# freewilll/doom-rust-renderer

Hardware: AMD Instinct MI355X
Metric: frames/sec (fixed e1m1 camera path) (higher is better)
Workload: dtype f32

## Files before the change

doom-rust-renderer_amd/csrc/context.cpp:

```cpp
#include <hip/hip_runtime_api.h>
#include <sched.h>

#include <algorithm>
#include <atomic>
#include <cstdlib>
#include <cstdio>
#include <cstring>
#include <chrono>
#include <memory>
#include <string>
#include <thread>
#include <vector>

#include "../../include/doomgpu.h"
#include "api_common.hpp"
#include "binner.hpp"
#include "fe_kernels.hpp"
#include "fs_kernels.hpp"
#include "light_fx_kernels.hpp"
#include "mobj_fx_kernels.hpp"
#include "frontend.hpp"
#include "hip_mem.hpp"
#include "kernels.hpp"
#include "map_kernels.hpp"
// ... 58 lines not shown
    DevPtr<uint32_t> d_flags;
    FeParams FP{};
    FsParams FSP{};
    LfxRows LR{};
    MfxRows MR{};
    int32_t front_end = DG_FE_HOST;
    void describe(int32_t fe, int n, uint64_t bytes, uint64_t walls, uint64_t planes) {
        front_end = fe; phase = Phase::Prepared; n_frames = n; list_bytes = bytes; n_walls = walls; n_planes = planes;
        max_spans = 0; n_spans = 0; covered = 0;
    }
    bool column_walk() const { return front_end == DG_FE_DEVICE || front_end == DG_FE_DEVICE_SEGS; }
    bool seg_walk() const { return front_end == DG_FE_DEVICE_SEGS; }
    bool harvested = true;
    bool map_built = false;
    std::vector<dg_view> views;
    std::vector<dg_view_state> states;
    std::vector<dg_sector_light> state_lights;
    std::vector<dg_mobj_state> state_mobjs;
    const Scene *snap_scene = nullptr;
    uint64_t snap_rev = 0;
    std::vector<dg_sector_light> snap_lights;
    std::vector<dg_mobj_state> snap_mobjs;
    void snapshot_scene(const Scene &sc) {
        if (snap_scene == &sc && snap_rev == sc.revision && snap_lights.size() == sc.sectors.size() && snap_mobjs.size() == sc.mobjs.size()) return;
        snap_lights.resize(sc.sectors.size()); snap_mobjs.resize(sc.mobjs.size());
        for (size_t i = 0; i < sc.sectors.size(); i++) snap_lights[i] = dg_sector_light{(int32_t)i, (int32_t)sc.sectors[i].light};
        for (size_t i = 0; i < sc.mobjs.size(); i++) snap_mobjs[i] = dg_mobj_state{(int32_t)i, sc.mobjs[i].sprite_frame, sc.mobjs[i].full_bright ? 1 : 0, 0};
        snap_scene = &sc; snap_rev = sc.revision;
    }
    struct RedoState { std::vector<dg_sector_light> lights; std::vector<dg_mobj_state> mobjs; dg_view_state st{}; };
    const dg_view_state *state_for_redo(const Scene &sc, int i, RedoState &tmp, const SceneFx &fx) const {
        const dg_view_state *own = states.empty() ? nullptr : &states[(size_t)i];
        if (snap_scene != &sc || snap_rev == sc.revision) return own;
        tmp.lights.clear();
        const bool lfx = fx.light.fits(sc), mfx = fx.mobj.fits(sc);
        for (const dg_sector_light &l : snap_lights)
            if (!lfx || fx.light.rec_of[(size_t)l.sector] < 0) tmp.lights.push_back(l);
        tmp.mobjs.clear();
        for (const dg_mobj_state &m : snap_mobjs)
            if (!mfx || fx.mobj.type_of[(size_t)m.mobj] < 0) tmp.mobjs.push_back(m);
        if (own) { tmp.lights.insert(tmp.lights.end(), own->lights, own->lights + own->n_lights); tmp.mobjs.insert(tmp.mobjs.end(), own->mobjs, own->mobjs + own->n_mobjs); }
        tmp.st = dg_view_state{tmp.lights.data(), (uint32_t)tmp.lights.size(), tmp.mobjs.data(), (uint32_t)tmp.mobjs.size()};
        return &tmp.st;
    }
    void keep_states(const dg_view_state *st, int n) {
        states.clear(); state_lights.clear(); state_mobjs.clear();
        if (!st) return;
        for (int i = 0; i < n; i++) { state_lights.insert(state_lights.end(), st[i].lights, st[i].lights + st[i].n_lights); state_mobjs.insert(state_mobjs.end(), st[i].mobjs, st[i].mobjs + st[i].n_mobjs); }
        size_t lo = 0, mo = 0;
        for (int i = 0; i < n; i++) {
            states.push_back(dg_view_state{state_lights.data() + lo, st[i].n_lights, state_mobjs.data() + mo, st[i].n_mobjs});
            lo += st[i].n_lights; mo += st[i].n_mobjs;
        }
    }
};

struct FeFrameOut {
    std::vector<FePart> parts;
    std::vector<FeSprite> sprites;
    std::vector<uint32_t> behind, sky_parts, bin_off, sbin_off;
    std::vector<uint16_t> bin_parts, sbin_sprites;
    uint32_t behind_words = 0, n_sky_slots = 0;
    DevFrame hdr{};
};

}

struct dg_ctx {
    dg_config cfg{};
    FrameConsts fk{};
    DevConsts dk{};
    const Scene *scene = nullptr;
    size_t uploaded_texels = 0;
    DevPtr<uint32_t> d_palette;
    DevPtr<uint8_t> d_texel_idx, d_texel_opq;
    uint8_t *d_flats = nullptr;
    DevPtr<unsigned long long> d_checksums;
    DevPtr<uint4> d_row_tab;
    DevScene dscene{};
    std::vector<Slot> slots;
    hipStream_t kstream = nullptr;
    hipStream_t rstream = nullptr;
    bool raster_overlap = false;
    std::unique_ptr<Pool> pool;
    std::vector<std::unique_ptr<FrameArena>> arenas;
    std::vector<BinnedFrame> binned;
    size_t span_cap_per_batch = 0, wall_cap_per_batch = 0, plane_cap_per_batch = 0;
    int n_threads = 1;
    bool fe_enabled = false;
    bool fe_scene_ok = false;
    bool fs_enabled = false, fs_scene_ok = false;
    bool fs_rows_dirty = true;
    bool preparing = false;
    bool fs_forced = false;
    double ema_host = -1.0, ema_gpu_dev = -1.0, ema_gpu_fs = -1.0;
    int host_samples = 0;
    int since_probe = 0;
    int since_fs_probe = 0;
    int gpu_samples[2] = {0, 0};
    DevPtr<uint8_t> d_fs_scene;
    SceneFx fx;
    DevPtr<uint8_t> d_wall_fx;
    FsFx fs_fx{};
    DevPtr<uint8_t> d_light_fx;
    LfxRows lfx_proto{};
    DevPtr<uint8_t> d_mobj_fx;
    MfxRows mfx_proto{};
    DevPtr<uint8_t> d_fs_scratch;
    size_t fs_zero_bytes = 0;
    FsParams fs_proto{};
    uint64_t fallbacks_fe = 0;
    uint64_t redone_frames = 0;
    DevPtr<DevRSpan> d_redo_rspans;
    size_t redo_span_cap = 0;
    std::vector<FeFrameOut> fe_out;
    uint32_t fe_col_slots = FE_DEFAULT_COL_SLOTS;
    size_t fe_part_cap = 0, fe_sprite_cap = 0, fe_behind_cap = 0, fe_bin_cap = 0, fe_sbin_cap = 0, fe_slab_cap = 0;
    DevPtr<uint32_t> d_fe_cnt;
    DevPtr<FeU4> d_fe_cspans;
    DevPtr<FeColRec> d_fe_recs;
    DevPtr<uint8_t> d_map_layer;
    bool map_layer_ok = false;
    DevPtr<uint8_t> d_walk_tables;
    const WalkNode *d_walk_nodes = nullptr;
    const WalkLeaf *d_walk_leaves = nullptr;
    hipStream_t wstream = nullptr;
    hipStream_t xstream = nullptr;
    hipEvent_t ev_reduce0 = nullptr, ev_reduce1 = nullptr;
    bool reduce_timed = false;
};

namespace {

int cgroup_cpu_quota() {
    long long quota = -1, period = 0;
    if (FILE *f = std::fopen("/sys/fs/cgroup/cpu.max", "r")) {
        char q[32] = {0};
        if (std::fscanf(f, "%31s %lld", q, &period) == 2 && std::strcmp(q, "max") != 0) quota = std::atoll(q);
        std::fclose(f);
    } else {
        if (FILE *g = std::fopen("/sys/fs/cgroup/cpu/cpu.cfs_quota_us", "r")) { if (std::fscanf(g, "%lld", &quota) != 1) quota = -1; std::fclose(g); }
        if (FILE *g = std::fopen("/sys/fs/cgroup/cpu/cpu.cfs_period_us", "r")) { if (std::fscanf(g, "%lld", &period) != 1) period = 0; std::fclose(g); }
    }
    if (quota <= 0 || period <= 0) return 0;
    return (int)((quota + period - 1) / period);
}

hipError_t slot_sync(Slot &s) {
    if (s.raster_recorded) { const hipError_t e = hipEventSynchronize(s.ev_raster); if (e != hipSuccess) return e; }
    return hipStreamSynchronize(s.stream);
}

void free_ctx(dg_ctx *c) {
    if (!c) return;
    (void)hipSetDevice(c->cfg.device);
    if (c->kstream) (void)hipStreamSynchronize(c->kstream);
    if (c->rstream) (void)hipStreamSynchronize(c->rstream);
    for (Slot &s : c->slots) {
        if (s.stream) (void)hipStreamSynchronize(s.stream);
        if (s.copy_stream) (void)hipStreamSynchronize(s.copy_stream);
        for (hipEvent_t ev : {s.ev_start, s.ev_setup, s.ev_raster, s.ev_rstart, s.ev_h2d})
            if (ev) (void)hipEventDestroy(ev);
        if (s.copy_stream) (void)hipStreamDestroy(s.copy_stream);
        if (s.stream) (void)hipStreamDestroy(s.stream);
    }
    if (c->kstream) (void)hipStreamDestroy(c->kstream);
    if (c->rstream) (void)hipStreamDestroy(c->rstream);
    if (c->wstream) { (void)hipStreamSynchronize(c->wstream); (void)hipStreamDestroy(c->wstream); }
    if (c->xstream) { (void)hipStreamSynchronize(c->xstream); (void)hipStreamDestroy(c->xstream); }
    for (hipEvent_t ev : {c->ev_reduce0, c->ev_reduce1})
        if (ev) (void)hipEventDestroy(ev);
    delete c;
}

int check_batch(const dg_ctx *c, int n) {
    if (!c->scene) return set_err(DG_ERR_INVALID, "no scene uploaded (dg_upload_scene)");
    if (n <= 0 || n > c->cfg.max_batch) return set_err(DG_ERR_CAPACITY, "batch size outside [1, max_batch]");
    if (c->scene->texel_idx.size() != c->uploaded_texels) return set_err(DG_ERR_INVALID, "the scene decoded new bitmaps since dg_upload_scene: upload it again");
    return DG_OK;
}

void pack_binned(uint8_t *h, const ListLayout &L, const BinnedFrame &bf, size_t i, size_t W) {
    std::memcpy(h + L.frames + i * sizeof(DevFrame), &bf.hdr, sizeof(DevFrame));
    std::memcpy(h + L.col_off + i * (W + 1) * 4, bf.col_off.data(), (W + 1) * 4);
    if (!bf.walls.empty()) std::memcpy(h + L.walls + (size_t)bf.hdr.wall_base * sizeof(DevWallRec), bf.walls.data(), bf.walls.size() * sizeof(DevWallRec));
    if (!bf.planes.empty()) std::memcpy(h + L.planes + (size_t)bf.hdr.plane_base * sizeof(DevPlaneRec), bf.planes.data(), bf.planes.size() * sizeof(DevPlaneRec));
    if (!bf.spans.empty()) std::memcpy(h + L.spans + (size_t)bf.hdr.span_base * sizeof(DevSpan), bf.spans.data(), bf.spans.size() * sizeof(DevSpan));
}

void point_at_lists(RasterParams &P, const uint8_t *d, const ListLayout &L) {
    P.frames = reinterpret_cast<const DevFrame *>(d + L.frames);
    P.col_off = reinterpret_cast<const uint32_t *>(d + L.col_off);
    P.walls = reinterpret_cast<const DevWallRec *>(d + L.walls);
    P.planes = reinterpret_cast<const DevPlaneRec *>(d + L.planes);
    P.spans = reinterpret_cast<const DevSpan *>(d + L.spans);
}

void fill_raster_params(dg_ctx *c, Slot &s, int n) {
    RasterParams &P = s.P;
    P.scene = c->dscene;
    P.k = c->dk;
    P.rspans = s.d_rspans.get();
    P.fb = s.d_fb.get();
    P.row_tab = c->d_row_tab.get();
    P.n_frames = n;
}

template <class T> void point_at(T *&p, uint8_t *d, size_t off) { p = reinterpret_cast<T *>(d + off); }
template <class Params, class Layout> void point_at_records(Params &P, uint8_t *d, const Layout &L) {
    point_at(P.fframes, d, L.fframes); point_at(P.parts, d, L.parts); point_at(P.sprites, d, L.sprites);
    point_at(P.behind, d, L.behind); point_at(P.sky_parts, d, L.sky);
    point_at(P.bin_off, d, L.bin_off); point_at(P.sbin_off, d, L.sbin_off); point_at(P.bin_parts, d, L.bins); point_at(P.sbin_sprites, d, L.sbins);
}

uint32_t fe_span_stride(const dg_ctx *c) { return (uint32_t)(c->span_cap_per_batch / (size_t)c->cfg.max_batch); }

void fill_walk_params(dg_ctx *c, Slot &s, int n) {
    FeParams &F = s.FP;
    F.scene = c->dscene;
    F.k = c->dk;
    F.cspans = c->d_fe_cspans.get(); F.recs = c->d_fe_recs.get(); F.cnt = c->d_fe_cnt.get();
    F.events = s.d_events;
    F.flags = s.d_flags.get();
    F.host_flags = s.h_status.get(); F.totals = s.h_status.get() + c->cfg.max_batch;
    F.col_off = s.d_fe_coloff.get(); F.rspans = s.d_rspans.get();
    F.n_frames = n; F.span_stride = fe_span_stride(c); F.w64 = (uint32_t)((c->cfg.width + 63) / 64); F.col_slots = c->fe_col_slots;
    fill_raster_params(c, s, n);
    s.P.frames = F.frames;
    s.P.col_off = s.d_fe_coloff.get();
    s.P.walls = nullptr; s.P.planes = nullptr; s.P.spans = nullptr;
}

int build_batch_host(dg_ctx *c, Slot &s, const dg_view *views, const dg_frame_lists *given, int n, const dg_view_state *states = nullptr) {
    const auto t0 = std::chrono::steady_clock::now();
    if (const int bad = check_batch(c, n)) return bad;
    const Scene &sc = *c->scene;
    const int W = c->cfg.width, H = c->cfg.height;
    std::vector<int> rc((size_t)n, 0);
    std::vector<std::string> errs((size_t)n);
    c->pool->parallel_for(n, [&](int i, int wid) {
        BinnedFrame &bf = c->binned[(size_t)i];
        if (given) {
            dg_frame_lists fl = given[i];
            fill_view_trig(fl.view);
            rc[(size_t)i] = bin_frame(sc, c->fk, fl, bf, errs[(size_t)i]);
        } else {
            dg_view v = views[i];
            fill_view_trig(v);
            dg_frame_lists fl;
            rc[(size_t)i] = build_frame_lists(sc, W, H, v, *c->arenas[(size_t)wid], fl, errs[(size_t)i], states ? &states[i] : nullptr, &c->fx);
            if (!rc[(size_t)i]) rc[(size_t)i] = bin_frame(sc, c->fk, fl, bf, errs[(size_t)i]);
        }
    });
    for (int i = 0; i < n; i++)
        if (rc[(size_t)i]) return set_err(rc[(size_t)i], "frame " + std::to_string(i) + ": " + errs[(size_t)i]);

    uint64_t spans = 0, walls = 0, planes = 0, covered = 0;
    uint32_t max_spans = 0;
    for (int i = 0; i < n; i++) {
        BinnedFrame &bf = c->binned[(size_t)i];
        bf.hdr.span_base = (uint32_t)spans; bf.hdr.wall_base = (uint32_t)walls; bf.hdr.plane_base = (uint32_t)planes;
        spans += bf.spans.size(); walls += bf.walls.size(); planes += bf.planes.size(); covered += bf.covered_pixels;
        max_spans = std::max<uint32_t>(max_spans, (uint32_t)bf.spans.size());
    }
    if (spans > c->span_cap_per_batch || walls > c->wall_cap_per_batch || planes > c->plane_cap_per_batch)
        return set_err(DG_ERR_CAPACITY, "frame lists exceed the slot's list slab");
    const ListLayout L = list_layout((size_t)n, (size_t)W, walls, planes, spans);
    if (L.total > s.lists_cap) return set_err(DG_ERR_CAPACITY, "list slab too small");
    c->pool->parallel_for(n, [&](int i, int) { pack_binned(s.h_lists.get(), L, c->binned[(size_t)i], (size_t)i, (size_t)W); });
    fill_raster_params(c, s, n);
    point_at_lists(s.P, s.d_lists.get(), L);
    s.describe(DG_FE_HOST, n, L.total, walls, planes);
    s.max_spans = max_spans; s.n_spans = spans; s.covered = covered;
    s.host_ms = std::chrono::duration<float, std::milli>(std::chrono::steady_clock::now() - t0).count();
    HIP_TRY(hipMemcpyAsync(s.d_lists.get(), s.h_lists.get(), L.total, hipMemcpyHostToDevice, s.stream));
    return DG_OK;
}

int build_batch_fe(dg_ctx *c, Slot &s, const dg_view *views, int n, const dg_view_state *states) {
    const auto t0 = std::chrono::steady_clock::now();
    if (const int bad = check_batch(c, n)) return bad;
    const Scene &sc = *c->scene;
    const int W = c->cfg.width, H = c->cfg.height;
    std::vector<int> rc((size_t)n, 0);
    std::vector<std::string> errs((size_t)n);
    c->pool->parallel_for(n, [&](int i, int wid) {
        FrameArena &A = *c->arenas[(size_t)wid];
        FeFrameOut &o = c->fe_out[(size_t)i];
// ... 535 lines not shown
}

}

extern "C" {

int dg_create(const dg_config *cfg, dg_ctx **out) {
    if (!cfg || !out) return set_err(DG_ERR_INVALID, "null argument");
    if (cfg->width <= 0 || cfg->height <= 0 || cfg->width > 16384 || cfg->height > 16384)
        return set_err(DG_ERR_INVALID, "width/height must be positive, both <= 16384");
    if (cfg->max_batch <= 0 || cfg->max_batch > 65535 || cfg->slots <= 0 || cfg->slots > 16)
        return set_err(DG_ERR_INVALID, "max_batch must be in [1, 65535], slots in [1, 16]");
    if (cfg->front_end < DG_FE_AUTO || cfg->front_end > DG_FE_DEVICE_SEGS) return set_err(DG_ERR_INVALID, "front_end must be DG_FE_AUTO, DG_FE_HOST, DG_FE_DEVICE or DG_FE_DEVICE_SEGS");
    int ndev = 0;
    if (hipGetDeviceCount(&ndev) != hipSuccess || ndev <= 0) return set_err(DG_ERR_NO_DEVICE, "no HIP device (this library has no CPU path)");
    if (cfg->device < 0 || cfg->device >= ndev) return set_err(DG_ERR_NO_DEVICE, "device ordinal out of range");
    hipDeviceProp_t prop;
    HIP_TRY(hipGetDeviceProperties(&prop, cfg->device));
    if (std::strncmp(prop.gcnArchName, "gfx950", 6) != 0)
        return set_err(DG_ERR_NO_DEVICE, std::string("device is ") + prop.gcnArchName + ", this build targets gfx950 only");
    HIP_TRY(hipSetDevice(cfg->device));

    dg_ctx *c = new dg_ctx();
    c->cfg = *cfg;
    c->fk = make_consts(cfg->width, cfg->height);
    c->dk = DevConsts{c->fk.ARC, c->fk.GCFX, c->fk.CFX, c->fk.CFY, cfg->width, cfg->height};
    int nthreads = cfg->host_threads;
    if (nthreads <= 0) {
        cpu_set_t set;
        CPU_ZERO(&set);
        int avail = sched_getaffinity(0, sizeof set, &set) == 0 ? CPU_COUNT(&set) : (int)std::thread::hardware_concurrency();
        const int quota = cgroup_cpu_quota();
        if (quota > 0) avail = std::min(avail, quota);
        nthreads = std::max(1, std::min(avail, 16));
    }
    nthreads = std::min(nthreads, 256);
    c->n_threads = nthreads;
    c->pool.reset(new Pool(nthreads - 1));
    for (int i = 0; i < nthreads; i++) c->arenas.emplace_back(new FrameArena());
    c->binned.resize((size_t)cfg->max_batch);

    const size_t W = (size_t)cfg->width, H = (size_t)cfg->height, F = (size_t)cfg->max_batch;
    c->span_cap_per_batch = F * W * 24;
    c->wall_cap_per_batch = F * 4096;
    c->plane_cap_per_batch = F * 4096;
    const size_t lists_cap = list_layout(F, W, c->wall_cap_per_batch, c->plane_cap_per_batch, c->span_cap_per_batch).total + 1024;
    c->fe_enabled = cfg->front_end != DG_FE_HOST;
    c->fs_enabled = cfg->front_end == DG_FE_DEVICE_SEGS || cfg->front_end == DG_FE_AUTO;
    c->fs_forced = cfg->front_end == DG_FE_DEVICE_SEGS;
    if (c->fe_enabled) {
        if (const char *e = std::getenv("DOOMGPU_FE_COLUMN_SLOTS")) {
            const long v = std::strtol(e, nullptr, 10);
            if (v >= 1 && v <= (long)FE_MAX_COL_SLOTS) c->fe_col_slots = (uint32_t)v;
        }
        c->fe_out.resize(F);
        size_t parts_per_frame = 2048;
        if (const char *e = std::getenv("DOOMGPU_FE_RECORDS_PER_FRAME")) {
            const long v = std::strtol(e, nullptr, 10);
            if (v >= 1 && v <= 65535) parts_per_frame = (size_t)v;
        }
        c->fe_part_cap = F * parts_per_frame;
        c->fe_sprite_cap = F * 256;
        c->fe_behind_cap = F * 256 * 32;
        c->fe_bin_cap = F * 16384;
        c->fe_sbin_cap = F * 2048;
        c->fe_slab_cap = fe_layout(F, W, c->fe_part_cap, c->fe_sprite_cap, c->fe_behind_cap, F * FE_MAX_SKY_SLOTS, c->fe_bin_cap, c->fe_sbin_cap).total + 1024;
    }
    c->slots.resize((size_t)cfg->slots);
    hipError_t e;
#define CTX_TRY(expr) if ((e = (expr)) != hipSuccess) { std::string m = std::string(#expr) + ": " + hipGetErrorString(e); free_ctx(c); return set_err(DG_ERR_HIP, m); }
    CTX_TRY(hip_alloc(c->d_checksums, F * 8));
    if (c->fe_enabled) {
        CTX_TRY(hip_alloc(c->d_fe_cspans, F * c->fe_col_slots * W * sizeof(FeU4)));
        CTX_TRY(hip_alloc(c->d_fe_recs, F * c->fe_col_slots * W * sizeof(FeColRec)));
        CTX_TRY(hip_alloc(c->d_fe_cnt, F * W * 4));
    }
    {
        int lo = 0, hi = 0;
        CTX_TRY(hipDeviceGetStreamPriorityRange(&lo, &hi));
        CTX_TRY(hipStreamCreateWithPriority(&c->kstream, hipStreamNonBlocking, hi));
        c->raster_overlap = (size_t)cfg->width * (size_t)cfg->height <= kOverlapMaxPixels;
        if (const char *e = std::getenv("DOOMGPU_RASTER_OVERLAP")) c->raster_overlap = std::atoi(e) != 0;
        if (c->raster_overlap) CTX_TRY(hipStreamCreateWithPriority(&c->rstream, hipStreamNonBlocking, hi));
    }
    for (Slot &s : c->slots) {
        CTX_TRY(hipStreamCreateWithFlags(&s.stream, hipStreamNonBlocking));
        for (hipEvent_t *ev : {&s.ev_start, &s.ev_setup, &s.ev_raster, &s.ev_rstart}) CTX_TRY(hipEventCreate(ev));
        CTX_TRY(hipEventCreateWithFlags(&s.ev_h2d, hipEventDisableTiming));
        CTX_TRY(hipStreamCreateWithFlags(&s.copy_stream, hipStreamNonBlocking));
        CTX_TRY(hip_alloc(s.h_lists, lists_cap));
        CTX_TRY(hip_alloc(s.d_lists, lists_cap));
        CTX_TRY(hip_alloc(s.d_rspans, c->span_cap_per_batch * sizeof(DevRSpan)));
        CTX_TRY(hip_alloc(s.d_fb, F * 3 * W * H));
        if (c->fe_enabled) {
            CTX_TRY(hip_alloc(s.h_fe, c->fe_slab_cap));
            CTX_TRY(hip_alloc(s.d_fe, c->fe_slab_cap));
            CTX_TRY(hip_alloc(s.d_fe_coloff, F * (W + 1) * 4));
            CTX_TRY(hip_alloc(s.d_order, FS_ORDER_CLASSES * F * fe_col_groups(W) * 4));
            SlabCursor ws;
            ws.take(F * 4 + FS_ORDER_CLASSES * 4);
            const size_t off_events = ws.take(F * FE_MAX_SKY_SLOTS * 3 * ((W + 63) / 64) * 8);
            s.walk_state_bytes = ws.end();
            CTX_TRY(hip_alloc(s.d_flags, s.walk_state_bytes));
            s.d_events = reinterpret_cast<uint64_t *>(reinterpret_cast<uint8_t *>(s.d_flags.get()) + off_events);
            CTX_TRY(hip_alloc(s.h_status, 2 * F * 4));
        }
        s.lists_cap = lists_cap;
    }
#undef CTX_TRY
    *out = c;
    return DG_OK;
}

void dg_destroy(dg_ctx *ctx) { free_ctx(ctx); }
int dg_ctx_host_threads(const dg_ctx *ctx) { return ctx ? ctx->n_threads : DG_ERR_INVALID; }

int dg_upload_scene(dg_ctx *c, const dg_scene *scene) {
    if (!c || !scene) return set_err(DG_ERR_INVALID, "null argument");
    HIP_TRY(hipSetDevice(c->cfg.device));
    for (Slot &s : c->slots) {
        if (c->scene) (void)take_slot(c, s);
        HIP_TRY(slot_sync(s));
        HIP_TRY(hipStreamSynchronize(s.copy_stream));
        s.copy_pending = false;
    }
    const Scene &sc = *scene->sc;
    c->d_palette.reset(); c->d_texel_idx.reset(); c->d_texel_opq.reset();
    c->d_flats = nullptr;
    for (Slot &s : c->slots) s.reset();
    c->d_walk_tables.reset();
    c->map_layer_ok = false;
    uint32_t pal[256];
    for (int i = 0; i < 256; i++) pal[i] = (uint32_t)sc.palette[3 * i] | ((uint32_t)sc.palette[3 * i + 1] << 8) | ((uint32_t)sc.palette[3 * i + 2] << 16);
    const size_t nt = std::max<size_t>(sc.texel_idx.size(), 16), nf = std::max<size_t>(sc.flat_pool.size(), 16);
    float palf[256 * 4];
    for (int i = 0; i < 256; i++) { palf[4 * i] = (float)sc.palette[3 * i]; palf[4 * i + 1] = (float)sc.palette[3 * i + 1]; palf[4 * i + 2] = (float)sc.palette[3 * i + 2]; palf[4 * i + 3] = 0.0f; }
    HIP_TRY(hip_alloc(c->d_palette, sizeof pal + sizeof palf));
    const size_t flats_at = (nt + 255) & ~(size_t)255;
    HIP_TRY(hip_alloc(c->d_texel_idx, flats_at + nf));
    HIP_TRY(hip_alloc(c->d_texel_opq, nt));
    c->d_flats = c->d_texel_idx.get() + flats_at;
    HIP_TRY(hipMemcpy(c->d_palette.get(), pal, sizeof pal, hipMemcpyHostToDevice));
    HIP_TRY(hipMemcpy(c->d_palette.get() + 256, palf, sizeof palf, hipMemcpyHostToDevice));
    if (!sc.texel_idx.empty()) {
        HIP_TRY(hipMemcpy(c->d_texel_idx.get(), sc.texel_idx.data(), sc.texel_idx.size(), hipMemcpyHostToDevice));
        HIP_TRY(hipMemcpy(c->d_texel_opq.get(), sc.texel_opq.data(), sc.texel_opq.size(), hipMemcpyHostToDevice));
    }
    if (!sc.flat_pool.empty()) HIP_TRY(hipMemcpy(c->d_flats, sc.flat_pool.data(), sc.flat_pool.size(), hipMemcpyHostToDevice));
    const BitmapInfo &sky = sc.bitmaps[(size_t)sc.sky_bitmap];
    c->dscene = DevScene{c->d_palette.get(), reinterpret_cast<const float *>(c->d_palette.get() + 256), c->d_texel_idx.get(), c->d_texel_opq.get(), c->d_flats, sky.texel_off, sky.w, sky.h, sky.has_holes};
    if (!c->d_row_tab) HIP_TRY(hip_alloc(c->d_row_tab, (size_t)c->cfg.height * sizeof(uint4)));
    HIP_TRY(launch_row_table(c->dscene, c->dk, c->d_row_tab.get(), nullptr));
    HIP_TRY(hipDeviceSynchronize());
    c->scene = &sc;
    c->fx = sc.fx;
    c->fe_scene_ok = sky.w >= 256 && sky.h >= 128;
    c->uploaded_texels = sc.texel_idx.size();
    c->fs_scene_ok = false;
    if (c->fs_enabled && c->fe_scene_ok && sc.fs_ok && c->cfg.width <= FS_MAX_W) {
        const int rc = upload_fs_scene(c, sc);
        if (rc && c->fs_forced) return rc;
        if (rc) {
            static bool said = false;
            if (!said) { said = true; std::fprintf(stderr, "doomgpu: DG_FE_AUTO keeps the per-seg half on the host: no device memory for the seg walk's per-batch rows (%d views x %zu segs)\n", c->cfg.max_batch, sc.segs.size()); }
            drop_fs_scene(c);
            c->fs_scene_ok = false;
// ... 345 lines not shown
```

doom-rust-renderer_amd/csrc/kernels.hip:

```cpp
#include <hip/hip_runtime.h>
#include <cstdlib>
#include <hip/hip_ext.h>

#include <algorithm>
#include <type_traits>

#include "kernels.hpp"
#include "raster_core.h"

namespace dg {

constexpr int TILE_W = 64;
constexpr int TILE_H = 64;
constexpr int WAVES = 8;
constexpr int THREADS = WAVES * 64;
constexpr int SPAN_CAP = 512;

__global__ __launch_bounds__(256) void dg_setup_spans(RasterParams P) {
    const int f = blockIdx.y;
    const DevFrame fr = P.frames[f];
    const uint32_t i = blockIdx.x * blockDim.x + threadIdx.x;
    if (i >= fr.n_spans) return;
    const DevSpan sp = P.spans[fr.span_base + i];
    DevRSpan o;
// ... 411 lines not shown
                C.winner = off;
            } else {
                if (big & colmask) {
                    const uint32_t n0 = bcast(f_n0, 8 * k), n = bcast(f_n, 8 * k);
                    C.winner = big_column_owner(L.lw0 + n0, 32u * (n0 + 1u), n, lane, y0, R);
                } else {
                    C.winner = owner_loop(hit_op & colmask, v_lo, v_rg, v_off, R, 0u);
                }
                o = owner_texel(T, L.lspans, C.winner, R, C.factor);
            }
            C.tex = P.scene.texel_idx[o];
        };
        auto stage2 = [&](int k, const Col &C) {
            const unsigned long long colmask = 0xffull << (8 * k);
            uint32_t tex = C.tex;
            float factor = C.factor;
            if (walk2 & colmask) {
                if (big & colmask) {
                    const uint32_t n0 = bcast(f_n0, 8 * k), n = bcast(f_n, 8 * k);
                    big_column_overlays(P, T, L.lw0 + n0, lspans_addr, 32u * (n0 + 1u), n, lane, y0, R, C.winner, tex, factor);
                } else {
                    overlay_loop(P, T, lspans_addr, hit_ov & colmask, v_lo, v_rg, v_off, R, C.winner, tex, factor);
                }
            }
            float4 c;
            asm volatile("ds_read_b128 %0, %1\n\ts_waitcnt lgkmcnt(0)" : "=v"(c) : "v"(pal_addr + (tex << 4)));
            tcol[k * WAVES * TILE_TS] = shade_f(c, factor);
        };
        Col A, B;
        if (nk == WAVES) {
            stage1(0, A);
#pragma unroll
            for (int k = 1; k < WAVES - 1; k += 2) {
                stage1(k, B);
                stage2(k - 1, A);
                stage1(k + 1, A);
                stage2(k, B);
            }
            stage1(WAVES - 1, B);
            stage2(WAVES - 2, A);
            stage2(WAVES - 1, B);
        } else {
            for (int k = 0; k < nk; k++) {
                stage1(k, A);
                stage2(k, A);
            }
        }

        c_lo = c_hi;
        if (c_lo < TILE_W) __syncthreads();
    }
    __syncthreads();

    const int gc = (lane & 7) | ((lane >> 5) << 3), rsub = (lane >> 3) & 3;
#pragma unroll
    for (int pass = 0; pass < TILE_H / (4 * WAVES); pass++) {
        const int row = pass * 4 * WAVES + wave * 4 + rsub;
        const int yy = y0 + row, xx = x0 + 4 * gc;
        if (yy < H && xx < W) {
            const uint32_t p0 = L.tile[(4 * gc + 0) * TILE_TS + row], p1 = L.tile[(4 * gc + 1) * TILE_TS + row];
            const uint32_t p2 = L.tile[(4 * gc + 2) * TILE_TS + row], p3 = L.tile[(4 * gc + 3) * TILE_TS + row];
            if constexpr (W4) {
                uint32_t *dst = reinterpret_cast<uint32_t *>(fb + ((size_t)yy * (size_t)W + (size_t)xx) * 3);
                __builtin_nontemporal_store((p0 & 0xffffffu) | (p1 << 24), dst + 0);
                __builtin_nontemporal_store(((p1 >> 8) & 0xffffu) | (p2 << 16), dst + 1);
                __builtin_nontemporal_store(((p2 >> 16) & 0xffu) | (p3 << 8), dst + 2);
            } else {
                uint8_t *dst = fb + ((size_t)yy * (size_t)W + (size_t)xx) * 3;
                const uint32_t px[4] = {p0, p1, p2, p3};
#pragma unroll
                for (int j = 0; j < 4; j++) {
                    if (xx + j >= W) break;
                    __builtin_nontemporal_store((uint8_t)px[j], dst + 3 * j + 0);
                    __builtin_nontemporal_store((uint8_t)(px[j] >> 8), dst + 3 * j + 1);
                    __builtin_nontemporal_store((uint8_t)(px[j] >> 16), dst + 3 * j + 2);
                }
            }
        }
    }
    if (ty + 1 < ty_end) __syncthreads();
  }
}

__device__ __forceinline__ void raster_block(const RasterParams &P, uint32_t &bx, uint32_t &by, uint32_t &f) {
    bx = blockIdx.x; by = blockIdx.y; f = blockIdx.z;
    if (!P.frame_per_xcd) return;
    const uint32_t gx = gridDim.x, gy = gridDim.y, pf = gx * gy;
    const uint32_t orig = bx + gx * (by + gy * f);
    if (orig >= ((uint32_t)P.n_frames & ~7u) * pf) return;
    const uint32_t xcd = orig & 7u, idx = orig >> 3;
    const uint32_t j = __umulhi(idx, P.xcd_rcp_pf), w = idx - j * pf;
    f = j * 8u + xcd;
    by = __umulhi(w, P.xcd_rcp_gx);
    bx = w - by * gx;
}

__global__ __launch_bounds__(THREADS, 8) void dg_raster_tiles(RasterParams P) {
    __shared__ __attribute__((aligned(16))) TileLds L;
    const int n_tile_rows = (P.k.H + TILE_H - 1) / TILE_H;
    uint32_t bx, by, f;
    raster_block(P, bx, by, f);
    const int ty_begin = (int)by * P.tile_rows_per_wg;
    strip_body<true>(P, L, (int)f, (int)bx * TILE_W, ty_begin, min(n_tile_rows, ty_begin + P.tile_rows_per_wg));
}
__global__ __launch_bounds__(THREADS, 8) void dg_raster_tiles_anyw(RasterParams P) {
    __shared__ __attribute__((aligned(16))) TileLds L;
    const int n_tile_rows = (P.k.H + TILE_H - 1) / TILE_H;
    uint32_t bx, by, f;
    raster_block(P, bx, by, f);
    const int ty_begin = (int)by * P.tile_rows_per_wg;
    strip_body<false>(P, L, (int)f, (int)bx * TILE_W, ty_begin, min(n_tile_rows, ty_begin + P.tile_rows_per_wg));
}

__global__ void dg_row_table(DevScene scene, DevConsts k, uint4 *row_tab) {
    const int y = (int)(blockIdx.x * blockDim.x + threadIdx.x);
    if (y >= k.H) return;
    const float vy = k.CFY - (float)y;
    const int32_t srow = sky_row(scene, k, y);
    row_tab[y] = make_uint4(f32_bits(prepare_rcp(vy)), f32_bits(vy), (srow < 0 ? 0u : (uint32_t)srow) | (vy != 0.0f ? 0x100u : 0u), f32_bits(srow < 0 ? 0.0f : 1.0f));
}

__global__ __launch_bounds__(256) void dg_checksum(const uint8_t *fb, size_t frame_bytes, unsigned long long *out) {
    const uint8_t *b = fb + (size_t)blockIdx.y * frame_bytes;
    const uint32_t *d = reinterpret_cast<const uint32_t *>(b);
    const bool dwords = (frame_bytes & 3) == 0;
    const size_t n = (frame_bytes + 3) / 4;
    unsigned long long acc = 0;
    for (size_t i = (size_t)blockIdx.x * blockDim.x + threadIdx.x; i < n; i += (size_t)gridDim.x * blockDim.x) {
        uint32_t v;
        if (dwords) v = d[i];
        else {
            v = 0;
            for (size_t k = 0; k < 4 && 4 * i + k < frame_bytes; k++) v |= (uint32_t)b[4 * i + k] << (8 * k);
        }
        unsigned long long m = ((unsigned long long)v ^ (i * 0x9E3779B97F4A7C15ull)) * 0xBF58476D1CE4E5B9ull;
        acc += m ^ (m >> 32);
    }
    for (int o = 32; o > 0; o >>= 1) acc += __shfl_down(acc, o);
    if ((threadIdx.x & 63) == 0) atomicAdd(&out[blockIdx.y], acc);
}

hipError_t launch_checksums(const uint8_t *fb, size_t frame_bytes, int count, unsigned long long *out, hipStream_t stream) {
    if (count <= 0) return hipSuccess;
    const unsigned blocks = (unsigned)std::min<size_t>(256, ((frame_bytes + 3) / 4 + 255) / 256);
    hipLaunchKernelGGL(dg_checksum, dim3(blocks, (unsigned)count), dim3(256), 0, stream, fb, frame_bytes, out);
    return hipGetLastError();
}

hipError_t launch_row_table(const DevScene &scene, const DevConsts &k, uint4 *row_tab, hipStream_t stream) {
    hipLaunchKernelGGL(dg_row_table, dim3((unsigned)((k.H + 255) / 256)), dim3(256), 0, stream, scene, k, row_tab);
    return hipGetLastError();
}

static hipError_t record_pair(hipStream_t stream, hipEvent_t start, hipEvent_t stop) {
    hipError_t e = hipSuccess;
    if (start) e = hipEventRecord(start, stream);
    if (e == hipSuccess && stop) e = hipEventRecord(stop, stream);
    return e;
}

hipError_t launch_setup(const RasterParams &P, uint32_t max_spans_per_frame, hipStream_t stream, hipEvent_t start, hipEvent_t stop) {
    if (P.n_frames <= 0 || max_spans_per_frame == 0) return record_pair(stream, start, stop);
    dim3 grid((max_spans_per_frame + 255) / 256, (unsigned)P.n_frames);
    hipExtLaunchKernelGGL(dg_setup_spans, grid, dim3(256), 0, stream, start, stop, 0, P);
    return hipGetLastError();
}

int raster_tile_rows_per_wg(int W, int H, int n_frames) {
    const int n_tile_rows = (H + TILE_H - 1) / TILE_H;
    if (n_tile_rows < 8) return std::min(2, n_tile_rows);
    const long long strips = (long long)((W + TILE_W - 1) / TILE_W) * (long long)std::max(1, n_frames);
    long long segments = (30000 + strips - 1) / strips;
    segments = std::max(1ll, std::min(segments, (long long)((n_tile_rows + 2) / 3)));
    return (int)((n_tile_rows + segments - 1) / segments);
}

hipError_t launch_raster(const RasterParams &P_in, hipStream_t stream, hipEvent_t start, hipEvent_t stop) {
    if (P_in.n_frames <= 0) return record_pair(stream, start, stop);
    RasterParams P = P_in;
    const int n_tile_rows = (P.k.H + TILE_H - 1) / TILE_H;
    if (P.tile_rows_per_wg <= 0) P.tile_rows_per_wg = raster_tile_rows_per_wg(P.k.W, P.k.H, P.n_frames);
    dim3 grid((unsigned)((P.k.W + TILE_W - 1) / TILE_W), (unsigned)((n_tile_rows + P.tile_rows_per_wg - 1) / P.tile_rows_per_wg), (unsigned)P.n_frames);
    P.frame_per_xcd = (size_t)P.k.W * (size_t)P.k.H <= 1100000 ? 1 : 0;
    if (const char *e = std::getenv("DOOMGPU_FRAME_PER_XCD")) P.frame_per_xcd = std::atoi(e) != 0 ? 1 : 0;
    {
        const uint64_t gx = grid.x, pf = (uint64_t)grid.x * grid.y, total = pf * grid.z;
        if (gx < 2 || total * pf >= (1ull << 32)) P.frame_per_xcd = 0;
        else { P.xcd_rcp_pf = (uint32_t)((1ull << 32) / pf + 1); P.xcd_rcp_gx = (uint32_t)((1ull << 32) / gx + 1); }
    }
    if (P.k.W % 4 == 0) hipExtLaunchKernelGGL(dg_raster_tiles, grid, dim3(THREADS), 0, stream, start, stop, 0, P);
    else hipExtLaunchKernelGGL(dg_raster_tiles_anyw, grid, dim3(THREADS), 0, stream, start, stop, 0, P);
    return hipGetLastError();
}

}
```

doom-rust-renderer_amd/csrc/kernels.hpp:

```cpp
#pragma once
#include <hip/hip_runtime_api.h>
#include <hip/hip_vector_types.h>

#include "lists_dev.h"

namespace dg {

struct RasterParams {
    DevScene scene;
    DevConsts k;
    const DevFrame *frames;
    const uint32_t *col_off;
    const DevSpan *spans;
    DevRSpan *rspans;
    const DevWallRec *walls;
    const DevPlaneRec *planes;
    uint8_t *fb;
    const uint4 *row_tab;
    int32_t n_frames;
    int32_t frame_per_xcd;
    uint32_t xcd_rcp_pf, xcd_rcp_gx;
    int32_t tile_rows_per_wg;
};

hipError_t launch_setup(const RasterParams &P, uint32_t max_spans_per_frame, hipStream_t stream, hipEvent_t start = nullptr, hipEvent_t stop = nullptr);
hipError_t launch_raster(const RasterParams &P, hipStream_t stream, hipEvent_t start = nullptr, hipEvent_t stop = nullptr);
hipError_t launch_checksums(const uint8_t *fb, size_t frame_bytes, int count, unsigned long long *out, hipStream_t stream);
hipError_t launch_row_table(const DevScene &scene, const DevConsts &k, uint4 *row_tab, hipStream_t stream);

}
```

Baseline: 559,800.

## Split raster grid into full-height long strips plus short tail segments

Replaces the uniform raster work-group mapping with a planner that can give most frames full-height column strips (one work-group per strip) and cut the remaining tail frames into short row segments, dealt across XCDs. The aim is to cut per-work-group overhead on the bulk of frames while keeping the GPU busy at the tail of the batch. The default rule turns the split on whenever the frame count leaves enough long strips. It adds index-decoding arithmetic per block and a debug export, and long strips risk load imbalance.

```diff
diff --git a/doom-rust-renderer_amd/csrc/context.cpp b/doom-rust-renderer_amd/csrc/context.cpp
--- a/doom-rust-renderer_amd/csrc/context.cpp
+++ b/doom-rust-renderer_amd/csrc/context.cpp
@@ -164,6 +164,7 @@
     hipStream_t kstream = nullptr;
     hipStream_t rstream = nullptr;
     bool raster_overlap = false;
+    RasterAsk raster_ask;
     std::unique_ptr<Pool> pool;
     std::vector<std::unique_ptr<FrameArena>> arenas;
     std::vector<BinnedFrame> binned;
@@ -286,6 +287,7 @@
     P.fb = s.d_fb.get();
     P.row_tab = c->d_row_tab.get();
     P.n_frames = n;
+    P.ask = c->raster_ask;
 }
 
 template <class T> void point_at(T *&p, uint8_t *d, size_t off) { p = reinterpret_cast<T *>(d + off); }
@@ -987,6 +989,15 @@
         c->raster_overlap = (size_t)cfg->width * (size_t)cfg->height <= kOverlapMaxPixels;
         if (const char *e = std::getenv("DOOMGPU_RASTER_OVERLAP")) c->raster_overlap = std::atoi(e) != 0;
         if (c->raster_overlap) CTX_TRY(hipStreamCreateWithPriority(&c->rstream, hipStreamNonBlocking, hi));
+        if (const char *e = std::getenv("DOOMGPU_FRAME_PER_XCD")) c->raster_ask.frame_per_xcd = std::atoi(e) != 0 ? 1 : 0;
+        if (const char *e = std::getenv("DOOMGPU_RASTER_SHAPE")) {
+            int n_long = 0, rows = 0;
+            if (!std::strcmp(e, "uniform")) c->raster_ask.shape = 1;
+            else if (!std::strcmp(e, "split")) c->raster_ask.shape = 2;
+            else if (std::sscanf(e, "split:%d:%d", &n_long, &rows) == 2 && n_long >= 0 && rows >= 1) {
+                c->raster_ask.shape = 2; c->raster_ask.n_long = n_long; c->raster_ask.short_rows = rows;
+            }
+        }
     }
     for (Slot &s : c->slots) {
         CTX_TRY(hipStreamCreateWithFlags(&s.stream, hipStreamNonBlocking));
diff --git a/doom-rust-renderer_amd/csrc/kernels.hip b/doom-rust-renderer_amd/csrc/kernels.hip
--- a/doom-rust-renderer_amd/csrc/kernels.hip
+++ b/doom-rust-renderer_amd/csrc/kernels.hip
@@ -517,34 +517,23 @@
   }
 }
 
-__device__ __forceinline__ void raster_block(const RasterParams &P, uint32_t &bx, uint32_t &by, uint32_t &f) {
-    bx = blockIdx.x; by = blockIdx.y; f = blockIdx.z;
-    if (!P.frame_per_xcd) return;
-    const uint32_t gx = gridDim.x, gy = gridDim.y, pf = gx * gy;
-    const uint32_t orig = bx + gx * (by + gy * f);
-    if (orig >= ((uint32_t)P.n_frames & ~7u) * pf) return;
-    const uint32_t xcd = orig & 7u, idx = orig >> 3;
-    const uint32_t j = __umulhi(idx, P.xcd_rcp_pf), w = idx - j * pf;
-    f = j * 8u + xcd;
-    by = __umulhi(w, P.xcd_rcp_gx);
-    bx = w - by * gx;
+__device__ __forceinline__ RasterBlock raster_block(const RasterMap &M) {
+    if (M.split) return raster_map_split(M, blockIdx.x);
+    const uint32_t orig = blockIdx.x + gridDim.x * (blockIdx.y + gridDim.y * blockIdx.z);
+    if (orig < M.b1) return raster_map_dealt(M, orig);
+    const int32_t ty = (int32_t)blockIdx.y * M.rows;
+    return RasterBlock{blockIdx.z, blockIdx.x, ty, min(M.n_tile_rows, ty + M.rows)};
 }
 
 __global__ __launch_bounds__(THREADS, 8) void dg_raster_tiles(RasterParams P) {
     __shared__ __attribute__((aligned(16))) TileLds L;
-    const int n_tile_rows = (P.k.H + TILE_H - 1) / TILE_H;
-    uint32_t bx, by, f;
-    raster_block(P, bx, by, f);
-    const int ty_begin = (int)by * P.tile_rows_per_wg;
-    strip_body<true>(P, L, (int)f, (int)bx * TILE_W, ty_begin, min(n_tile_rows, ty_begin + P.tile_rows_per_wg));
+    const RasterBlock b = raster_block(P.map);
+    strip_body<true>(P, L, (int)b.f, (int)b.bx * TILE_W, b.ty_begin, b.ty_end);
 }
 __global__ __launch_bounds__(THREADS, 8) void dg_raster_tiles_anyw(RasterParams P) {
     __shared__ __attribute__((aligned(16))) TileLds L;
-    const int n_tile_rows = (P.k.H + TILE_H - 1) / TILE_H;
-    uint32_t bx, by, f;
-    raster_block(P, bx, by, f);
-    const int ty_begin = (int)by * P.tile_rows_per_wg;
-    strip_body<false>(P, L, (int)f, (int)bx * TILE_W, ty_begin, min(n_tile_rows, ty_begin + P.tile_rows_per_wg));
+    const RasterBlock b = raster_block(P.map);
+    strip_body<false>(P, L, (int)b.f, (int)b.bx * TILE_W, b.ty_begin, b.ty_end);
 }
 
 __global__ void dg_row_table(DevScene scene, DevConsts k, uint4 *row_tab) {
@@ -601,31 +590,35 @@
     return hipGetLastError();
 }
 
-int raster_tile_rows_per_wg(int W, int H, int n_frames) {
-    const int n_tile_rows = (H + TILE_H - 1) / TILE_H;
-    if (n_tile_rows < 8) return std::min(2, n_tile_rows);
-    const long long strips = (long long)((W + TILE_W - 1) / TILE_W) * (long long)std::max(1, n_frames);
-    long long segments = (30000 + strips - 1) / strips;
-    segments = std::max(1ll, std::min(segments, (long long)((n_tile_rows + 2) / 3)));
-    return (int)((n_tile_rows + segments - 1) / segments);
-}
+int raster_tile_rows_per_wg(int W, int H, int n_frames) { return raster_uniform_rows(W, H, n_frames); }
 
 hipError_t launch_raster(const RasterParams &P_in, hipStream_t stream, hipEvent_t start, hipEvent_t stop) {
     if (P_in.n_frames <= 0) return record_pair(stream, start, stop);
     RasterParams P = P_in;
-    const int n_tile_rows = (P.k.H + TILE_H - 1) / TILE_H;
-    if (P.tile_rows_per_wg <= 0) P.tile_rows_per_wg = raster_tile_rows_per_wg(P.k.W, P.k.H, P.n_frames);
-    dim3 grid((unsigned)((P.k.W + TILE_W - 1) / TILE_W), (unsigned)((n_tile_rows + P.tile_rows_per_wg - 1) / P.tile_rows_per_wg), (unsigned)P.n_frames);
-    P.frame_per_xcd = (size_t)P.k.W * (size_t)P.k.H <= 1100000 ? 1 : 0;
-    if (const char *e = std::getenv("DOOMGPU_FRAME_PER_XCD")) P.frame_per_xcd = std::atoi(e) != 0 ? 1 : 0;
-    {
-        const uint64_t gx = grid.x, pf = (uint64_t)grid.x * grid.y, total = pf * grid.z;
-        if (gx < 2 || total * pf >= (1ull << 32)) P.frame_per_xcd = 0;
-        else { P.xcd_rcp_pf = (uint32_t)((1ull << 32) / pf + 1); P.xcd_rcp_gx = (uint32_t)((1ull << 32) / gx + 1); }
-    }
+    uint32_t g[3];
+    P.map = raster_plan(P.k.W, P.k.H, P.n_frames, P.tile_rows_per_wg, P.ask, g);
+    const dim3 grid(g[0], g[1], g[2]);
     if (P.k.W % 4 == 0) hipExtLaunchKernelGGL(dg_raster_tiles, grid, dim3(THREADS), 0, stream, start, stop, 0, P);
     else hipExtLaunchKernelGGL(dg_raster_tiles_anyw, grid, dim3(THREADS), 0, stream, start, stop, 0, P);
     return hipGetLastError();
 }
 
-}
+extern "C" uint32_t dg_debug_raster_plan(int W, int H, int n_frames, int tile_rows_per_wg, const int32_t *ask4, uint32_t *map_out, uint32_t *out, uint32_t cap) {
+    RasterAsk ask;
+    if (ask4) { ask.frame_per_xcd = ask4[0]; ask.shape = ask4[1]; ask.n_long = ask4[2]; ask.short_rows = ask4[3]; }
+    uint32_t g[3];
+    const RasterMap M = raster_plan(W, H, n_frames, tile_rows_per_wg, ask, g);
+    const uint32_t n = g[0] * g[1] * g[2];
+    if (map_out) {
+        const uint32_t m[18] = {(uint32_t)M.split, (uint32_t)M.frame_per_xcd, (uint32_t)M.rows, (uint32_t)M.n_tile_rows, M.gx, M.pf, M.rcp_gx, M.rcp_pf,
+                                M.b0, M.b1, M.nlx, M.lr, M.n_long, M.f2, g[0], g[1], g[2], n};
+        std::copy(m, m + 18, map_out);
+    }
+    for (uint32_t b = 0; out && b < n && b < cap; b++) {
+        const RasterBlock r = raster_map_any(M, b);
+        out[4 * b] = r.f; out[4 * b + 1] = r.bx; out[4 * b + 2] = (uint32_t)r.ty_begin; out[4 * b + 3] = (uint32_t)r.ty_end;
+    }
+    return n;
+}
+
+}
diff --git a/doom-rust-renderer_amd/csrc/kernels.hpp b/doom-rust-renderer_amd/csrc/kernels.hpp
--- a/doom-rust-renderer_amd/csrc/kernels.hpp
+++ b/doom-rust-renderer_amd/csrc/kernels.hpp
@@ -3,6 +3,7 @@
 #include <hip/hip_vector_types.h>
 
 #include "lists_dev.h"
+#include "raster_map.h"
 
 namespace dg {
 
@@ -18,9 +19,9 @@
     uint8_t *fb;
     const uint4 *row_tab;
     int32_t n_frames;
-    int32_t frame_per_xcd;
-    uint32_t xcd_rcp_pf, xcd_rcp_gx;
     int32_t tile_rows_per_wg;
+    RasterAsk ask;
+    RasterMap map;
 };
 
 hipError_t launch_setup(const RasterParams &P, uint32_t max_spans_per_frame, hipStream_t stream, hipEvent_t start = nullptr, hipEvent_t stop = nullptr);
diff --git a/doom-rust-renderer_amd/csrc/raster_map.h b/doom-rust-renderer_amd/csrc/raster_map.h
--- /dev/null
+++ b/doom-rust-renderer_amd/csrc/raster_map.h
@@ -0,0 +1,147 @@
+#pragma once
+#include <algorithm>
+#include <cstdint>
+
+#include "rust_num.h"
+
+namespace dg {
+
+constexpr int RASTER_TILE = 64;
+constexpr uint32_t RASTER_WG_SLOTS = 1024;
+constexpr uint64_t RASTER_MAX_GRID_X = 1u << 23;
+
+struct RasterAsk {
+    int32_t frame_per_xcd = -1;
+    int32_t shape = 0;
+    int32_t n_long = -1;
+    int32_t short_rows = 0;
+};
+
+struct RasterMap {
+    int32_t split;
+    int32_t frame_per_xcd;
+    int32_t rows;
+    int32_t n_tile_rows;
+    uint32_t gx, pf;
+    uint32_t rcp_gx, rcp_pf;
+    uint32_t b0, b1;
+    uint32_t nlx;
+    uint32_t lr, n_long, f2;
+};
+
+struct RasterBlock { uint32_t f, bx; int32_t ty_begin, ty_end; };
+
+DG_HD uint32_t raster_mulhi(uint32_t a, uint32_t b) { return (uint32_t)(((uint64_t)a * (uint64_t)b) >> 32); }
+
+DG_HD uint32_t raster_div(uint32_t n, uint32_t rcp) { return rcp ? raster_mulhi(n, rcp) : n; }
+DG_HD uint32_t raster_rcp(uint64_t d) { return d > 1 ? (uint32_t)((1ull << 32) / d + 1) : 0u; }
+
+DG_HD RasterBlock raster_segment(const RasterMap &M, uint32_t f, uint32_t bx, uint32_t seg) {
+    const int32_t ty = (int32_t)seg * M.rows;
+    return RasterBlock{f, bx, ty, ty + M.rows < M.n_tile_rows ? ty + M.rows : M.n_tile_rows};
+}
+DG_HD RasterBlock raster_short_item(const RasterMap &M, uint32_t f, uint32_t w) {
+    const uint32_t seg = raster_div(w, M.rcp_gx);
+    return raster_segment(M, f, w - seg * M.gx, seg);
+}
+
+DG_HD RasterBlock raster_map_dealt(const RasterMap &M, uint32_t b) {
+    const uint32_t xcd = b & 7u, idx = b >> 3;
+    const uint32_t j = raster_mulhi(idx, M.rcp_pf), w = idx - j * M.pf, seg = raster_mulhi(w, M.rcp_gx);
+    return raster_segment(M, j * 8u + xcd, w - seg * M.gx, seg);
+}
+
+DG_HD RasterBlock raster_map_split(const RasterMap &M, uint32_t b) {
+    if (b >= M.b1) {
+        const uint32_t c = b - M.b1, j = raster_div(c, M.rcp_pf);
+        return raster_short_item(M, M.f2 + j, c - j * M.pf);
+    }
+    uint32_t f, idx;
+    if (b < M.b0) { f = M.lr; idx = b; }
+    else {
+        const uint32_t c = b - M.b0, xcd = c & 7u;
+        idx = c >> 3;
+        if (idx >= M.nlx) {
+            idx -= M.nlx;
+            const uint32_t j = raster_div(idx, M.rcp_pf);
+            return raster_short_item(M, M.n_long + j * 8u + xcd, idx - j * M.pf);
+        }
+        f = xcd;
+    }
+    const uint32_t j = raster_div(idx, M.rcp_gx);
+    return RasterBlock{f + (b < M.b0 ? j : j * 8u), idx - j * M.gx, 0, M.n_tile_rows};
+}
+
+inline int raster_uniform_rows(int W, int H, int n_frames) {
+    const int n_tile_rows = (H + RASTER_TILE - 1) / RASTER_TILE;
+    if (n_tile_rows < 8) return std::min(2, n_tile_rows);
+    const long long strips = (long long)((W + RASTER_TILE - 1) / RASTER_TILE) * (long long)std::max(1, n_frames);
+    long long segments = (30000 + strips - 1) / strips;
+    segments = std::max(1ll, std::min(segments, (long long)((n_tile_rows + 2) / 3)));
+    return (int)((n_tile_rows + segments - 1) / segments);
+}
+
+constexpr uint32_t RASTER_TAIL_STRIPS = RASTER_WG_SLOTS * 9 / 4, RASTER_MIN_LONG_STRIPS = 2 * RASTER_WG_SLOTS;
+inline bool raster_split_rule(int W, int H, int n_frames, int &n_long, int &short_rows) {
+    const int n_tile_rows = (H + RASTER_TILE - 1) / RASTER_TILE, gx = (W + RASTER_TILE - 1) / RASTER_TILE;
+    n_long = 0; short_rows = std::min(n_tile_rows < 8 ? 2 : 3, n_tile_rows);
+    if (n_tile_rows < 7) return false;
+    const long long tail = (RASTER_TAIL_STRIPS + gx - 1) / gx, want = ((long long)n_frames - tail) & ~7ll;
+    if (want <= 0 || want * gx < (long long)RASTER_MIN_LONG_STRIPS) return false;
+    n_long = (int)want;
+    return true;
+}
+
+inline RasterMap raster_plan(int W, int H, int n_frames, int tile_rows_per_wg, const RasterAsk &ask, uint32_t grid[3]) {
+    RasterMap M{};
+    M.n_tile_rows = (H + RASTER_TILE - 1) / RASTER_TILE;
+    M.gx = (uint32_t)((W + RASTER_TILE - 1) / RASTER_TILE);
+    M.frame_per_xcd = ask.frame_per_xcd >= 0 ? (ask.frame_per_xcd ? 1 : 0) : (size_t)W * (size_t)H <= 1100000 ? 1 : 0;
+    int n_long = 0, short_rows = 0;
+    bool split = tile_rows_per_wg <= 0 && ask.shape != 1 && raster_split_rule(W, H, n_frames, n_long, short_rows);
+    if (tile_rows_per_wg <= 0 && ask.shape == 2 && ask.n_long >= 0) {
+        split = true;
+        n_long = std::min(ask.n_long, n_frames);
+        short_rows = std::max(1, std::min(ask.short_rows, M.n_tile_rows));
+    }
+    if (split) {
+        M.rows = short_rows;
+        const uint64_t segs = (uint64_t)((M.n_tile_rows + M.rows - 1) / M.rows), pf = M.gx * segs;
+        const uint64_t total = (uint64_t)n_long * M.gx + (uint64_t)(n_frames - n_long) * pf;
+        if (total >= RASTER_MAX_GRID_X || total * pf >= (1ull << 32)) split = false;
+        else {
+            M.split = 1;
+            M.pf = (uint32_t)pf;
+            M.rcp_pf = raster_rcp(pf); M.rcp_gx = raster_rcp(M.gx);
+            if (M.gx < 2) M.frame_per_xcd = 0;
+            M.n_long = (uint32_t)n_long;
+            M.lr = M.frame_per_xcd ? (uint32_t)n_long & ~7u : 0u;
+            const uint32_t s8 = M.frame_per_xcd ? (uint32_t)(n_frames - n_long) & ~7u : 0u;
+            M.f2 = M.n_long + s8;
+            M.nlx = M.lr / 8u * M.gx;
+            M.b0 = (M.n_long - M.lr) * M.gx;
+            M.b1 = M.b0 + 8u * (M.nlx + s8 / 8u * M.pf);
+            grid[0] = (uint32_t)total; grid[1] = 1; grid[2] = 1;
+            return M;
+        }
+    }
+    M.rows = tile_rows_per_wg > 0 ? tile_rows_per_wg : raster_uniform_rows(W, H, n_frames);
+    const uint32_t gy = (uint32_t)((M.n_tile_rows + M.rows - 1) / M.rows);
+    const uint64_t pf = (uint64_t)M.gx * gy, total = pf * (uint64_t)n_frames;
+    M.pf = (uint32_t)pf;
+    if (M.gx < 2 || total * pf >= (1ull << 32)) M.frame_per_xcd = 0;
+    else { M.rcp_pf = raster_rcp(pf); M.rcp_gx = raster_rcp(M.gx); }
+    M.b1 = M.frame_per_xcd ? ((uint32_t)n_frames & ~7u) * M.pf : 0u;
+    grid[0] = M.gx; grid[1] = gy; grid[2] = (uint32_t)n_frames;
+    return M;
+}
+
+inline RasterBlock raster_map_any(const RasterMap &M, uint32_t b) {
+    if (M.split) return raster_map_split(M, b);
+    if (b < M.b1) return raster_map_dealt(M, b);
+    const uint32_t f = b / M.pf, w = b % M.pf, seg = w / M.gx;
+    const int32_t ty = (int32_t)seg * M.rows;
+    return RasterBlock{f, w % M.gx, ty, std::min(M.n_tile_rows, ty + M.rows)};
+}
+
+}
```

New measurement: 577,500 (median of 6 runs). +3.2%, better.
